# brdav/refign

Measured on AMD Instinct MI355X. Metric: image-pairs/s (align+seg fwd+bwd, 1080x1920), higher is better.
Workload: dtype bf16

## Files before the change

### include/refign_hip.h

```cpp
#ifndef REFIGN_HIP_H
#define REFIGN_HIP_H

#ifdef __cplusplus
extern "C" {
#endif

#define RFN_OK 0
#define RFN_EINVAL (-1)
#define RFN_ELAUNCH (-2)
#define RFN_ENOTSUP (-3)
#define RFN_ENONDET (-4)

#define RFN_ABI_VERSION 5

typedef void* rfn_stream_t;

int rfn_abi_version(void);
const char* rfn_last_error(void);

int rfn_set_deterministic(int on);
int rfn_get_deterministic(void);

int rfn_corr_fwd_f32(const float* in1, const float* in2, float* out, int B, int C, int iH, int iW,
                     int kH, int kW, int patchH, int patchW, int padH, int padW, int dilH, int dilW,
// ... 185 lines not shown
int rfn_bn_apply_fwd(const void* x, const float* gamma, const float* beta, void* y, const double* sums, float* running_mean,
                     float* running_var, long T, int C, float eps, float momentum, int relu, int dtype, rfn_stream_t stream);
int rfn_bn_apply_fwd_ld(const void* x, const float* gamma, const float* beta, void* y, long ld_y, const double* sums,
                        float* running_mean, float* running_var, long T, int C, float eps, float momentum, int relu, int dtype,
                        rfn_stream_t stream);
int rfn_bn_stats_bwd(const void* x, const void* grad_y, const double* fwd_sums, const float* gamma, const float* beta,
                     float* bwd_sums, long T, int C, float eps, int relu, int dtype, rfn_stream_t stream);
int rfn_bn_apply_bwd(const void* x, const void* grad_y, const double* fwd_sums, const float* bwd_sums, const float* gamma,
                     const float* beta, void* grad_x, long T, int C, float eps, int relu, int dtype, rfn_stream_t stream);
int rfn_bn_train_fwd(const void* x, const float* gamma, const float* beta, void* y, double* sums, float* running_mean,
                     float* running_var, long T, int C, float eps, float momentum, int relu, int dtype,
                     rfn_stream_t stream);
int rfn_bn_train_bwd(const void* x, const void* grad_y, const double* fwd_sums, const float* gamma, const float* beta,
                     void* grad_x, float* bwd_sums, long T, int C, float eps, int relu, int dtype, rfn_stream_t stream);

int rfn_upsample_ce(const void* logits, const long* target, const float* weight, float* grad_lo, double* loss_sum, int B,
                    int C, int h, int w, int H, int W, int ignore_index, int dtype, int round16, rfn_stream_t stream);

int rfn_slide_argmax_confmat(const void* crop_logits, int dtype, int B, int C, int h, int w, const int* boxes, int nbox, int H,
                             int W, const long* target, int ignore_index, unsigned char* labels, long* confmat,
                             rfn_stream_t stream);

int rfn_gemm_nt_o32(const void* X, const void* W, const float* bias, const float* res, const float* rowscale,
                    int rows_per_sample, int act, float* Y, long M, long N, long K, long ldx, long ldw, long ldy,
                    rfn_stream_t stream);
int rfn_conv2d_nhwc_o32(const void* X, const void* W, const float* bias, int act, float* Y, int B, int H, int Wd, int C, int N,
                        int KH, int KW, int stride, int pad, int dil, long ldw, long ldy, int transposed,
                        rfn_stream_t stream);
int rfn_conv2d_nhwc_dgrad(const void* GY, const void* Wt, void* DX, int B, int H, int W, int C, int N, int KH, int KW,
                          int stride, int pad, int dil, long ldw, long ldy, int dtype, rfn_stream_t stream);
int rfn_conv2d_nhwc_wgrad(const void* GY, const void* X, float* P, float* grad_bias, int B, int H, int W, int C, int N, int KH,
                          int KW, int stride, int pad, int dil, long ldg, long Kpad, int rows_per_slab, int accumulate,
                          int dtype, rfn_stream_t stream);

int rfn_dacs_mix_jitter(const float* src, const float* trg, const long* gt_src, const long* pseudo_label,
                        const float* pseudo_weight, float* mixed_img, long* mixed_lbl, float* mixed_weight, double* mean_ws,
                        int B, int H, int W, const long* class_bits, const int* jitter_on, const int* order,
                        const float* factor, const float* hue, const float* mean3, const float* std3,
                        rfn_stream_t stream);
int rfn_dacs_blur(const float* x, float* tmp, float* y, int B, int C, int H, int W, int ksize_y, int ksize_x, const int* blur_on,
                  const double* sigma_y, const double* sigma_x, rfn_stream_t stream);

int rfn_crop_label_hist_u8(const void* label, int H, int W, const int* boxes, int K, int* hist, rfn_stream_t stream);
int rfn_crop_flip_norm_u8(const void* image, const void* label, int C, int H, int W, int top, int left, int h, int w, int flip,
                          const float* mean3, const float* std3, float* out_image, long* out_label, rfn_stream_t stream);

int rfn_resize_crop_flip_norm_u8(const void* image_hwc, int H, int W, int Hd, int Wd, const int* bounds_x, const int* coef_x, int kmax_x,
                                 const int* bounds_y, const int* coef_y, int kmax_y, int top, int left, int h, int w, int flip,
                                 const float* mean3, const float* std3, float* out_image, rfn_stream_t stream);
int rfn_resize_u8(const void* image_hwc, int H, int W, int Hd, int Wd, const int* bounds_x, const int* coef_x, int kmax_x,
                  const int* bounds_y, const int* coef_y, int kmax_y, void* out_chw, rfn_stream_t stream);
int rfn_resize_nearest_u8(const void* label, int H, int W, int Hd, int Wd, const int* ytab, const int* xtab, void* out,
                          rfn_stream_t stream);

int rfn_resize_filter_u8(const void* image_hwc, int H, int W, int Hd, int Wd, int filter, const int* bounds_x, const int* coef_x,
                         int kmax_x, const int* bounds_y, const int* coef_y, int kmax_y, void* out_chw, rfn_stream_t stream);
int rfn_resize_filter_crop_flip_norm_pad_u8(const void* image_hwc, int H, int W, int Hd, int Wd, int filter, const int* bounds_x,
                                            const int* coef_x, int kmax_x, const int* bounds_y, const int* coef_y, int kmax_y, int top,
                                            int left, int h, int w, int flip, const float* mean3, const float* std3, float* out_image,
                                            int Hf, int Wf, rfn_stream_t stream);

int rfn_sparse_epe_f32(const float* flow, const float* conf, const float* pts_src, const float* pts_trg, const int* offsets, int B,
                       int h, int w, double* rows, rfn_stream_t stream);

int rfn_gemm_nt_f8(const void* X8, const void* W8, const float* wscale, float x_scale, const void* bias, const void* res,
                   const float* rowscale, int rows_per_sample, int act, void* Y, int out_f8, float out_q, long M, long N,
                   long K, long ldx, long ldw, long ldy, rfn_stream_t stream);
int rfn_quant_rows_f8(const void* table, int nchunks, rfn_stream_t stream);
int rfn_quant_f8(const void* x_bf16, void* y8, long n, float q, rfn_stream_t stream);
int rfn_layernorm_fwd_f8(const void* x_bf16, const float* gamma, const float* beta, void* y8, long rows, int C, float eps,
                         float out_q, rfn_stream_t stream);
int rfn_dwconv3x3_gelu_nhwc_fwd_f8(const void* x8, const float* weight, const float* bias, void* y8, int B, int H, int W, int C,
                                   float x_scale, float out_q, rfn_stream_t stream);
int rfn_attn_pack_f8(const void* kv8, long batch_stride, long row_stride, int B, int heads, int Nkv, int nst, void* pack,
                     rfn_stream_t stream);
int rfn_attn_fwd_f8(const void* q8, long q_batch_stride, long q_row_stride, const void* pack, void* o8, long o_batch_stride,
                    long o_row_stride, int B, int heads, int Nq, int Nkv, int nst, float scale, float q_scale, float k_scale,
                    float v_scale, float out_q, rfn_stream_t stream);

unsigned long rfn_bn_stats_det_workspace_bytes(long T, int C);
int rfn_bn_stats_fwd_det(const void* x, double* sums, void* workspace, long T, int C, int dtype, rfn_stream_t stream);
int rfn_bn_stats_bwd_det(const void* x, const void* grad_y, const double* fwd_sums, const float* gamma, const float* beta,
                         float* bwd_sums, void* workspace, long T, int C, float eps, int relu, int dtype, rfn_stream_t stream);
unsigned long rfn_dwconv3x3_stats_det_workspace_bytes(int B, int H, int W, int C, int dilation);
int rfn_dwconv3x3_nhwc_fwd_stats_det(const void* x, const float* weight, const float* bias, void* y, double* sums, void* workspace,
                                     int B, int H, int W, int C, int dilation, int dtype, rfn_stream_t stream);
int rfn_dwconv3x3_nhwc_stats_det(const void* x, const float* weight, const float* bias, double* sums, void* workspace, int B, int H,
                                 int W, int C, int dilation, int dtype, rfn_stream_t stream);
int rfn_attn_bwd_dkv_det(const void* K, const void* V, long kv_batch_stride, long kv_row_stride, const void* q_rpack,
                         const void* q_tpack, const void* do_rpack, const void* do_tpack, const float* lse2,
                         const float* delta, float* accT, void* dKV, int B, int heads, int Nq, int Nkv, int nqblk, int nqpad,
                         int nkpad, int blocks_per_chunk, float scale, int dtype, rfn_stream_t stream);
unsigned long rfn_dacs_mix_jitter_det_workspace_bytes(int H, int W);
int rfn_dacs_mix_jitter_det(const float* src, const float* trg, const long* gt_src, const long* pseudo_label,
                            const float* pseudo_weight, float* mixed_img, long* mixed_lbl, float* mixed_weight, double* mean_ws,
                            int B, int H, int W, const long* class_bits, const int* jitter_on, const int* order,
                            const float* factor, const float* hue, const float* mean3, const float* std3,
                            rfn_stream_t stream);
unsigned long rfn_upsample_ce_det_workspace_bytes(int B, int C, int H, int W);
int rfn_upsample_ce_det(const void* logits, const long* target, const float* weight, float* grad_lo, double* loss_sum,
                        void* workspace, int B, int C, int h, int w, int H, int W, int ignore_index, int dtype, int round16,
                        rfn_stream_t stream);
int rfn_upsample_bilinear2d_bwd(const void* grad_out, void* grad_in, long planes, int h, int w, int H, int W, float scale_y,
                                float scale_x, int dtype, rfn_stream_t stream);

int rfn_steplog_gather(const void* const* ptrs, const int* dtypes, int n, double* row, rfn_stream_t stream);
int rfn_grad_sqnorm_groups(const float* flat, long n, const long* chunks, int nchunks, int ngroups, double* partials,
                           double* out, rfn_stream_t stream);

int rfn_grad_clip_coef(const double* sqnorms, int ngroups, float max_norm, float* coef, rfn_stream_t stream);
int rfn_grad_scale_f32(float* grads, long n, const float* coef, rfn_stream_t stream);
int rfn_grad_clamp_f32(float* grads, long n, float clip_value, rfn_stream_t stream);
int rfn_amp_unscale_sqnorm_groups_f32(float* grads, long n, const long* chunks, int nchunks, int ngroups, const float* scale,
                                      float* found_inf, double* partials, double* out, rfn_stream_t stream);

int rfn_flowsynth_flow_f32(const float* theta, int kind, const float* bumps, int n_bumps, const float* field, int h, int w,
                           float* flow, int* count, rfn_stream_t stream);
int rfn_flowsynth_warp_f32(const float* image, const float* flow, const int* count, int h, int w, int top, int left, int ch, int cw,
                           double min_fraction_valid, float* out_image, float* out_flow, void* out_mask, rfn_stream_t stream);
int rfn_gaussian_blur_f32(const float* src, const float* taps, int ntaps, int planes, int h, int w, double* tmp, float* dst,
                          rfn_stream_t stream);

int rfn_flowloss_block_pixels(void);
int rfn_flowloss_fwd_f32(const float* gt_flow, int B, int H, int W, const long* levels, const double* weights, int nlevels,
                         int loss_type, float delta, double* partials, int nblocks, float* loss_out, double* counts,
                         rfn_stream_t stream);
int rfn_flowloss_bwd_f32(const float* gt_flow, int B, int H, int W, const long* levels, const double* weights, int nlevels,
                         int loss_type, float delta, const double* counts, const float* grad_out, rfn_stream_t stream);
int rfn_multi_adam_f32(const void* table, int nchunks, const float* group_args, int ngroups, rfn_stream_t stream);
int rfn_multi_adam_amp_f32(const void* table, int nchunks, const double* group_args, int ngroups, const float* found_inf,
                           const float* step, rfn_stream_t stream);

int rfn_photometric_record_words(void);
int rfn_photometric_gray_sums_u8(const void* image, const void* records, int B, int h, int w, unsigned long* sums,
                                 rfn_stream_t stream);
int rfn_photometric_apply_u8(const void* image, const void* records, const unsigned long* sums, int B, int h, int w, float* out,
                             rfn_stream_t stream);

int rfn_rotate_nearest_u8(const void* src, int C, int H, int W, int a0, int a1, int a2, int a3, int a4, int a5, int fill,
                          void* out, void* outside, rfn_stream_t stream);
int rfn_photometric_gray_sums_geom_u8(const void* image, const void* records, const void* geom, int B, int H, int W, int h, int w,
                                      unsigned long* sums, rfn_stream_t stream);
int rfn_photometric_apply_geom_u8(const void* image, const void* records, const void* geom, const unsigned long* sums, int B, int H,
                                  int W, int h, int w, float* out, rfn_stream_t stream);

unsigned long rfn_warp_bwd_det_workspace_bytes(int B, int C, int H, int W, int want_grad_x, int want_grad_flow);
int rfn_warp_bwd_det_f32(const float* x, const float* flow, const float* grad_out, float* grad_x, float* grad_flow,
                         void* workspace, int B, int C, int H, int W, rfn_stream_t stream);
int rfn_corr_bwd_gather_f32(const float* in1, const float* in2, const float* grad_out, float* grad_in1,
                            float* grad_in2, int B, int C, int iH, int iW, int kH, int kW, int patchH, int patchW,
                            int padH, int padW, int dilH, int dilW, int dpH, int dpW, int dH, int dW,
                            rfn_stream_t stream);

#ifdef __cplusplus
}
#endif
#endif
```

### refign_amd/seg.py

```python
import math
import os
import random
from functools import partial, wraps
from typing import Callable, List, Optional, Union

import torch
import torch.nn as nn
import torch.nn.functional as F

from . import f8 as _f8
from . import linear as _linear
from . import determinism, mfma
from ._tensor import const_tensor
from ._tensor import DTYPE_CODE as _CE_DT
from .align import BaseHead
from .conv import Conv2d, patch_conv_tokens
from .layernorm import LayerNorm
from .layers import MLP, ConvBNReLU, DropPath
from .linear import Linear
from .upcat import upsample_concat
from .upsample import interpolate_bilinear

_MIT = {
    'mit_b0': ([32, 64, 160, 256], [2, 2, 2, 2]),
    'mit_b1': ([64, 128, 320, 512], [2, 2, 2, 2]),
    'mit_b2': ([64, 128, 320, 512], [3, 4, 6, 3]),
    'mit_b3': ([64, 128, 320, 512], [3, 4, 18, 3]),
    'mit_b4': ([64, 128, 320, 512], [3, 8, 27, 3]),
    'mit_b5': ([64, 128, 320, 512], [3, 6, 40, 3]),
}
_MIT_HEADS = [1, 2, 5, 8]
_MIT_SR = [8, 4, 2, 1]


_GRAD_READY_CB = None


class _GradMark(torch.autograd.Function):

    @staticmethod
    def forward(ctx, x, tag):
        ctx.tag = tag
        return x.view_as(x)

    @staticmethod
    def backward(ctx, g):
        cb = _GRAD_READY_CB
        if cb is not None:
            cb(ctx.tag)
        return g, None


def grad_mark(x, tag):
    return _GradMark.apply(x, tag) if (torch.is_grad_enabled() and x.requires_grad) else x


class DWConv(nn.Module):

    def __init__(self, dim=768):
        super().__init__()
        self.dwconv = nn.Conv2d(dim, dim, 3, 1, 1, bias=True, groups=dim)

    def forward(self, x, H, W):
        B, N, C = x.shape
        if x.is_cuda and C % 8 == 0:
            from .dwconv import dwconv3x3_tokens
            return dwconv3x3_tokens(x, self.dwconv.weight, self.dwconv.bias, H, W)
        y = self.dwconv(x.transpose(1, 2).reshape(B, C, H, W))
        return y.flatten(2).transpose(1, 2)


class Mlp(nn.Module):

    def __init__(self, in_features, hidden_features=None, out_features=None, act_layer=nn.GELU, drop=0.):
        super().__init__()
        out_features = out_features or in_features
        hidden_features = hidden_features or in_features
        self.fc1 = Linear(in_features, hidden_features)
        self.dwconv = DWConv(hidden_features)
        self.act = act_layer()
        self.fc2 = Linear(hidden_features, out_features)
        self.drop = nn.Dropout(drop)

    def forward(self, x, H, W, res=None, rowscale=None):
        if x.is_cuda and not torch.is_grad_enabled() and x.dtype in (torch.bfloat16, torch.float16) and type(self.act) is nn.GELU \
                and self.act.approximate == 'none' and self.drop.p == 0. and type(self.fc1) is Linear and not _f8.active():
            from .dwconv import ffn_fc1_dw_gelu
            a = ffn_fc1_dw_gelu(x, self.fc1, self.dwconv.dwconv, H, W)
            if a is not None:
                return self.fc2(a, res=res, rowscale=rowscale) if res is not None else self.fc2(a)
        x = self.fc1(x)
        if x.is_cuda and x.shape[-1] % 8 == 0 and type(self.act) is nn.GELU and self.act.approximate == 'none':
            from .dwconv import dwconv3x3_gelu_tokens
            dw = self.dwconv.dwconv
            if torch.is_grad_enabled() and x.requires_grad and self.drop.p == 0. and x.dtype in (torch.bfloat16, torch.float16) \
                    and os.environ.get("RFN_FUSED_GELU_BWD", "1") == "1":
                a, z = dwconv3x3_gelu_tokens(x, dw.weight, dw.bias, H, W, with_z=True)
                if res is not None:
                    return self.fc2(a, res=res, rowscale=rowscale, z=z)
                return self.fc2(a, z=z)
            x = self.drop(dwconv3x3_gelu_tokens(x, dw.weight, dw.bias, H, W))
        else:
            x = self.drop(self.act(self.dwconv(x, H, W)))
        if res is not None and self.drop.p == 0.:
            return self.fc2(x, res=res, rowscale=rowscale)
        y = self.drop(self.fc2(x))
        return y if res is None else _residual(res, y, rowscale)


_SDPA_BACKEND = None
_FUSED_UPCAT = True


def _fused_upcat_here():
    return _FUSED_UPCAT
_SR_AS_LINEAR = True
_KV_FUSED = True


class Attention(nn.Module):

    def __init__(self, dim, num_heads=8, qkv_bias=False, qk_scale=None, attn_drop=0., proj_drop=0., sr_ratio=1):
        super().__init__()
        assert dim % num_heads == 0, f'dim {dim} should be divided by num_heads {num_heads}.'
        self.dim, self.num_heads = dim, num_heads
        self.scale = qk_scale or (dim // num_heads) ** -0.5
        self.q = Linear(dim, dim, bias=qkv_bias)
        self.kv = Linear(dim, dim * 2, bias=qkv_bias)
        self.attn_drop = nn.Dropout(attn_drop)
        self.proj = Linear(dim, dim)
        self.proj_drop = nn.Dropout(proj_drop)
        self.sr_ratio = sr_ratio
        if sr_ratio > 1:
            self.sr = Conv2d(dim, dim, kernel_size=sr_ratio, stride=sr_ratio)
            self.norm = LayerNorm(dim)

    def forward(self, x, H, W, res=None, rowscale=None, x_kv=None):
        B, N, C = x.shape
        h, d = self.num_heads, C // self.num_heads
        q = self.q(x)
        if x_kv is not None:
            x = x_kv
        p = self.attn_drop.p if self.training else 0.0
        if _KV_FUSED and not torch.is_grad_enabled() and x.is_cuda and d == 64 and p == 0.0 and _SDPA_BACKEND is None \
                and q.dtype == x.dtype and type(self.kv) is Linear and not _f8.active() \
                and (self.sr_ratio == 1 or (_SR_AS_LINEAR and type(self.norm) is LayerNorm)):
            packs = mfma.kv_packs(x, H, W, self.sr if self.sr_ratio > 1 else None, self.norm if self.sr_ratio > 1 else None,
                                  self.kv)
            o = mfma.attention_packed(q, packs, h, self.scale) if packs is not None else None
            if o is not None:
                return self._project(o, res, rowscale)
        if self.sr_ratio > 1:
            r = patch_conv_tokens(x, H, W, self.sr) if _SR_AS_LINEAR else None
            if r is None:
                r = self.sr(x.transpose(1, 2).reshape(B, C, H, W)).flatten(2).transpose(1, 2)
            x = self.norm(r)
        kv = self.kv(x)
        o = mfma.attention(q, kv, h, self.scale) if (d == 64 and p == 0.0 and _SDPA_BACKEND is None) else None
        if o is None and q.is_cuda and q.dtype == torch.float32 and p == 0.0 and _SDPA_BACKEND is None:
            from . import split32
            if split32.usable(q, kv) and d in (32, 64):
                o = split32.attention(q, kv, h, self.scale)
        if o is None:
            mfma.note_library("sdpa", q, kv)
            q = q.view(B, N, h, d).transpose(1, 2)
# ... 325 lines not shown

class SegFormerHead(BaseHead):

    os: int = 4

    def __init__(self, in_channels: List[int], in_index: Union[List[int], int], num_classes: int,
                 input_transform: Optional[str] = None, channels: int = 256, dropout_ratio: float = 0.1):
        super().__init__(num_classes, in_index, input_transform)
        self.in_channels = in_channels
        c1, c2, c3, c4 = in_channels
        self.linear_c4 = MLP(input_dim=c4, embed_dim=channels)
        self.linear_c3 = MLP(input_dim=c3, embed_dim=channels)
        self.linear_c2 = MLP(input_dim=c2, embed_dim=channels)
        self.linear_c1 = MLP(input_dim=c1, embed_dim=channels)
        self.linear_fuse = ConvBNReLU(channels * 4, channels, kernel_size=1, norm_layer=nn.BatchNorm2d)
        self.linear_pred = nn.Conv2d(channels, num_classes, kernel_size=1)
        self.dropout = nn.Dropout2d(dropout_ratio) if dropout_ratio > 0 else None
        nn.init.normal_(self.linear_pred.weight, mean=0, std=0.01)
        nn.init.zeros_(self.linear_pred.bias)
        _mmseg_init(self)

    def forward(self, inputs):
        c1, c2, c3, c4 = inputs
        size = c1.shape[2:]

        feats = [c4, c3, c2, c1]
        toks = [layer(f) for layer, f in zip((self.linear_c4, self.linear_c3, self.linear_c2, self.linear_c1), feats)]
        cat = upsample_concat(toks, [f.shape[2:] for f in feats], size) if _fused_upcat_here() else None
        if cat is None:
            parts = []
            for t, f in zip(toks, feats):
                n, _, h, w = f.shape
                t = t.transpose(1, 2).reshape(n, -1, h, w)
                parts.append(t if (h, w) == tuple(size) else _up(t, size))
            cat = torch.cat(parts, dim=1)
        y = self.linear_fuse(cat)
        if self.dropout is not None:
            y = self.dropout(y)
        return _class_logits(self.linear_pred, y)


_PREDRAWN_CROPS = []
_DEVICE_CROPS = []


class DeviceBox:

    def __init__(self, off, h, w, divisible):
        self.off, self.h, self.w, self.divisible = off, int(h), int(w), int(divisible)

    def _idx(self, n, which, scale=1):
        return torch.arange(n, device=self.off.device) + self.off[which] // scale

    def crop(self, x):
        return x.index_select(-2, self._idx(self.h, 0)).index_select(-1, self._idx(self.w, 1))

    def mask(self, H, W, scale, like):
        assert self.divisible % int(scale) == 0
        hs, ws = int(self.h / scale), int(self.w / scale)
        ry = torch.arange(H, device=self.off.device) - self.off[0] // int(scale)
        rx = torch.arange(W, device=self.off.device) - self.off[1] // int(scale)
        m = ((ry >= 0) & (ry < hs))[:, None] & ((rx >= 0) & (rx < ws))[None, :]
        return m.to(like.dtype).view(1, 1, H, W)

    def insert(self, patch, size, scale):
        assert self.divisible % int(scale) == 0
        H, W = size
        hs, ws = patch.shape[-2:]
        ry = torch.arange(H, device=self.off.device) - self.off[0] // int(scale)
        rx = torch.arange(W, device=self.off.device) - self.off[1] // int(scale)
        ry = torch.where((ry >= 0) & (ry < hs), ry, torch.full_like(ry, hs))
        rx = torch.where((rx >= 0) & (rx < ws), rx, torch.full_like(rx, ws))
        return F.pad(patch, (0, 1, 0, 1)).index_select(-2, ry).index_select(-1, rx)


def push_device_crop(off, divisible):
    _DEVICE_CROPS.append((off, divisible))


def draw_crop_offsets(H, W, crop_size, divisible=1):
    if H == crop_size[-2] and W == crop_size[-1]:
        return None
    oy = random.randrange(0, int((max(H - crop_size[-2], 0) + 1) // divisible)) * divisible
    ox = random.randrange(0, int((max(W - crop_size[-1], 0) + 1) // divisible)) * divisible
    return int(oy), int(ox)


def predraw_crop(H, W, crop_size, divisible=1):
    _PREDRAWN_CROPS.append(((H, W, tuple(crop_size), divisible), draw_crop_offsets(H, W, crop_size, divisible)))


def extract_crop(img, crop_size, divisible=1):
    H, W = img.shape[-2:]
    assert crop_size[0] > 0 and crop_size[1] > 0
    if _DEVICE_CROPS:
        off, div = _DEVICE_CROPS.pop(0)
        assert div == divisible, (div, divisible)
        box = DeviceBox(off, crop_size[0], crop_size[1], divisible)
        return box.crop(img), [box]
    if _PREDRAWN_CROPS:
        key, off = _PREDRAWN_CROPS.pop(0)
        assert key == (H, W, tuple(crop_size), divisible), (key, (H, W, tuple(crop_size), divisible))
    else:
        off = draw_crop_offsets(H, W, crop_size, divisible)
    if off is None:
        return (0, H, 0, W)
    oy, ox = off
    y1, y2, x1, x2 = int(oy), int(oy + crop_size[0]), int(ox), int(ox + crop_size[1])
    return img[:, :, y1:y2, x1:x2], [[y1, y2, x1, x2]]


def scale_box(box, scale):
    return tuple(int(v / scale) for v in box)


def hr_crop_slice(crop_box, scale):
    y1, y2, x1, x2 = scale_box(crop_box, scale)
    return slice(y1, y2), slice(x1, x2)


def extract_slide_crop(img, crop_size):
    hc, wc = crop_size
    hs, ws = hc // 2, wc // 2
    H, W = img.shape[-2:]
    crops, boxes = [], []
    for iy in range(max(H - hc + hs - 1, 0) // hs + 1):
        for ix in range(max(W - wc + ws - 1, 0) // ws + 1):
            y2, x2 = min(iy * hs + hc, H), min(ix * ws + wc, W)
            y1, x1 = max(y2 - hc, 0), max(x2 - wc, 0)
            crops.append(img[:, :, y1:y2, x1:x2])
            boxes.append([y1, y2, x1, x2])
    return torch.cat(crops, dim=0), boxes


def hrda_backbone(self, head_os: int, is_teacher: bool = False) -> Callable:
    def deco(fn: Callable) -> Callable:
        @wraps(fn)
        def inner(x, *args, **kwargs):
            lr = F.interpolate(x, scale_factor=0.5, mode='bilinear', align_corners=False)
            size = lr.shape[-2:]
            if self.training and not is_teacher:
                hr, boxes = extract_crop(x, size, head_os * 2.0)
            else:
                hr, boxes = extract_slide_crop(x, size)
            nl, nh = lr.shape[0], hr.shape[0]
            feats = fn(torch.cat((lr, hr)), *args, **kwargs)
            lr_feats, hr_feats = zip(*(torch.split(f, [nl, nh]) for f in feats))
            return lr_feats, hr_feats, boxes
        return inner
    return deco


_REJOIN = True


def _rejoin(a, b):
    if _REJOIN and (not torch.is_grad_enabled() or not (a.requires_grad or b.requires_grad)) and a.dim() >= 2 \
            and a.dtype == b.dtype \
            and a.shape[1:] == b.shape[1:] and a.stride() == b.stride() and a.device == b.device \
            and a.untyped_storage().data_ptr() == b.untyped_storage().data_ptr() \
            and b.storage_offset() == a.storage_offset() + a.shape[0] * a.stride(0):
        dense = sorted(zip(a.stride()[1:], a.shape[1:]))
        run = 1
        for st, n in dense:
            if n != 1 and st != run:
                return torch.cat((a, b))
            run *= n
        if a.stride(0) == run:
            return a.as_strided((a.shape[0] + b.shape[0], *a.shape[1:]), a.stride(), a.storage_offset())
    return torch.cat((a, b))


def hrda_head(self, hrda_scale_attention: nn.Module, head_os: int, is_teacher: bool = False) -> Callable:
    def deco(fn: Callable) -> Callable:
        @wraps(fn)
        def inner(inp, *args, **kwargs):
            lr_feats, hr_feats, boxes = inp
            att = torch.sigmoid(hrda_scale_attention(lr_feats))
            nl, nh = lr_feats[0].shape[0], hr_feats[0].shape[0]
            seg = fn([_rejoin(*p) for p in zip(lr_feats, hr_feats)], *args, **kwargs)
            lr_seg, hr_seg = torch.split(seg, [nl, nh])
            if self.training and not is_teacher and isinstance(boxes[0], DeviceBox):
                box = boxes[0]
                att = att * box.mask(lr_seg.shape[2], lr_seg.shape[3], 2.0 * head_os, lr_seg)
                up_lr = interpolate_bilinear((1 - att) * lr_seg, scale_factor=2)
                up_att = interpolate_bilinear(att, scale_factor=2)
                inserted = box.insert(hr_seg, up_lr.shape[2:], head_os)
                return up_att * inserted + up_lr, defer_logits(hr_seg, (box.h, box.w), fused_ce_consumer(self)), box
            if self.training and not is_teacher:
                box = boxes[0]
                crop_size = (box[1] - box[0], box[3] - box[2])
                mask = lr_seg.new_zeros([nl, 1, *lr_seg.shape[2:]])
                sy, sx = hr_crop_slice(box, 2.0 * head_os)
                mask[:, :, sy, sx] = 1
                att = att * mask
                up_lr = interpolate_bilinear((1 - att) * lr_seg, scale_factor=2)
                up_att = interpolate_bilinear(att, scale_factor=2)
                inserted = torch.zeros_like(up_lr)
                sy, sx = hr_crop_slice(box, head_os)
                inserted[:, :, sy, sx] = hr_seg
                hr_logits = defer_logits(hr_seg, crop_size, fused_ce_consumer(self))
                return up_att * inserted + up_lr, hr_logits, box
            up_lr = F.interpolate((1 - att) * lr_seg, scale_factor=2, mode='bilinear', align_corners=False)
            for i in range(len(boxes)):
                boxes[i] = scale_box(boxes[i], head_os)
            Hh, Ww = max(b[1] for b in boxes), max(b[3] for b in boxes)
            preds = lr_seg.new_zeros((nl, self.num_classes, Hh, Ww))
            count = lr_seg.new_zeros((nl, 1, Hh, Ww))
            for i, (y1, y2, x1, x2) in enumerate(boxes):
                preds[:, :, y1:y2, x1:x2] += hr_seg[i * nl:(i + 1) * nl]
                count[:, :, y1:y2, x1:x2] += 1
            up_att = F.interpolate(att, scale_factor=2, mode='bilinear', align_corners=False)
            return up_att * (preds / count) + up_lr
        return inner
    return deco


_FUSED_CE = True


def mark_fused_ce_consumer(module, loss):
    module._rfn_fused_ce_consumer = type(loss) is PixelWeightedCrossEntropyLoss
    return module._rfn_fused_ce_consumer


def fused_ce_consumer(module):
    return bool(getattr(module, "_rfn_fused_ce_consumer", False))


class DeferredUpsample:

    def __init__(self, logits, size):
        self.logits, self.size = logits, (int(size[0]), int(size[1]))

    def materialize(self):
        return _up_logits(self.logits, self.size)

    @property
    def shape(self):
        return torch.Size((*self.logits.shape[:2], *self.size))

    @classmethod
    def __torch_function__(cls, func, types, args=(), kwargs=None):
        conv = lambda a: a.materialize() if isinstance(a, DeferredUpsample) else a
        return func(*[conv(a) for a in args], **{k: conv(v) for k, v in (kwargs or {}).items()})


def defer_logits(logits, size, consumer_is_fused_ce=False):
    if _FUSED_CE and consumer_is_fused_ce and logits.is_cuda and logits.dim() == 4 and logits.dtype in _CE_DT and logits.shape[1] <= 19 \
            and size[0] >= 2 * logits.shape[2] and size[1] >= 2 * logits.shape[3] and torch.is_grad_enabled():
        return DeferredUpsample(logits, size)
    return _up_logits(logits, size)


class _UpsampleCEFn(torch.autograd.Function):

    @staticmethod
    def forward(ctx, logits, target, weight, size, ignore_index):
        from . import _lib
        from ._tensor import ptr
        B, C, h, w = logits.shape
        H, W = size
        lg = logits.contiguous()
        tg = target.contiguous()
        wt = None if weight is None else weight.to(torch.float32).contiguous()
        if tg.dtype != torch.int64 or tuple(tg.shape) != (B, H, W) or (wt is not None and tuple(wt.shape) != (B, H, W)):
            raise RuntimeError("upsample_ce: target (B, H, W) int64 / weight (B, H, W) expected")
        grad = torch.empty((B, C, h, w), dtype=torch.float32, device=lg.device)
        total = torch.empty(64, dtype=torch.float64, device=lg.device)
        rc = None
        lib = _lib.load_library()
        if determinism.enabled():
            from ._tensor import workspace
            ws = workspace(lib.rfn_upsample_ce_det_workspace_bytes(B, C, H, W), lg.device)
            _lib.call("rfn_upsample_ce_det", lg.device, ptr(lg), ptr(tg), ptr(wt), ptr(grad), ptr(total), ptr(ws), B, C, h, w,
                      H, W, int(ignore_index), _CE_DT[lg.dtype], 1)
            ctx.save_for_backward(grad)
            ctx.npix, ctx.dtype = float(B * H * W), logits.dtype
            return (total[0] / ctx.npix).to(torch.float32)
        _lib.call("rfn_upsample_ce", lg.device, ptr(lg), ptr(tg), ptr(wt), ptr(grad), ptr(total), B, C, h, w, H, W,
                  int(ignore_index), _CE_DT[lg.dtype], 1)
        ctx.save_for_backward(grad)
        ctx.npix, ctx.dtype = float(B * H * W), logits.dtype
        return (total.sum() / ctx.npix).to(torch.float32)

    @staticmethod
    def backward(ctx, g):
        (grad,) = ctx.saved_tensors
        return (grad * (g.to(torch.float32) / ctx.npix)).to(ctx.dtype), None, None, None, None


class PixelWeightedCrossEntropyLoss(nn.Module):

    def __init__(self, ignore_index: int = 255) -> None:
        super().__init__()
        self.ignore_index = ignore_index

    def forward(self, input, target, pixel_weight=None):
        if isinstance(input, DeferredUpsample):
            if pixel_weight is not None:
                assert pixel_weight.dim() == target.dim()
            return _UpsampleCEFn.apply(input.logits, target, pixel_weight, input.size, self.ignore_index)
        loss = F.cross_entropy(input, target, ignore_index=self.ignore_index, reduction='none')
        if pixel_weight is not None:
            assert pixel_weight.dim() == loss.dim()
            loss = loss * pixel_weight.to(loss.dtype)
        return loss.mean()
```

Measured before the change: 17.42.

## Fuse HRDA attention-merge tail into single forward and backward kernels

Adds HIP kernels that take the raw scale-attention logits, lr and hr segmentation maps and produce the merged high-resolution logits in one pass. Sigmoid, crop mask, bilinear upsampling, crop insertion and blend are computed per output element instead of through a chain of separate PyTorch elementwise and interpolate ops. A matching fused backward kernel does the same for training, plus a fused sliding-window merge for the teacher/eval path. This removes many full-resolution intermediate tensors and kernel launches, at the cost of per-pixel recomputation, float64 accumulation in backward, and float32 channels-last output.

```diff
diff --git a/include/refign_hip.h b/include/refign_hip.h
--- a/include/refign_hip.h
+++ b/include/refign_hip.h
@@ -361,6 +361,17 @@
                             int padH, int padW, int dilH, int dilW, int dpH, int dpW, int dH, int dW,
                             rfn_stream_t stream);
 
+int rfn_hrda_merge_slide(const void* a, const long* a_strides, const void* lr, const long* lr_strides, const void* hr,
+                         const long* hr_strides, const int* boxes, int nb, float* out, int nl, int K, int h, int w, int hc, int wc,
+                         int dtype, int* accepted, rfn_stream_t stream);
+int rfn_hrda_fuse_crop_fwd(const void* a, const long* a_strides, const void* lr, const long* lr_strides, const void* hr,
+                           const long* hr_strides, const long* off, float* out, int n, int K, int h, int w, int hc, int wc, int mh,
+                           int mw, int div_mask, int div_ins, int dtype, rfn_stream_t stream);
+int rfn_hrda_fuse_crop_bwd(const float* grad_out, const long* g_strides, const void* a, const long* a_strides, const void* lr,
+                           const long* lr_strides, const void* hr, const long* hr_strides, const long* off, void* grad_a,
+                           void* grad_lr, void* grad_hr, int n, int K, int h, int w, int hc, int wc, int mh, int mw, int div_mask,
+                           int div_ins, int dtype, rfn_stream_t stream);
+
 #ifdef __cplusplus
 }
 #endif
diff --git a/refign_amd/csrc/hrdatail.hip b/refign_amd/csrc/hrdatail.hip
--- /dev/null
+++ b/refign_amd/csrc/hrdatail.hip
@@ -0,0 +1,291 @@
+#include <hip/hip_bf16.h>
+
+#include "bilinear.h"
+#include "common.h"
+#include "elem.h"
+
+namespace rfn {
+
+constexpr int kHrdaMaxBoxes = 16;
+
+struct HrdaMap {
+  const void* p;
+  long sn, sc, sh, sw;
+};
+struct HrdaBoxes {
+  int nb;
+  int y1[kHrdaMaxBoxes], y2[kHrdaMaxBoxes], x1[kHrdaMaxBoxes], x2[kHrdaMaxBoxes];
+};
+
+template <typename T>
+__device__ __forceinline__ float hrda_ld(const HrdaMap& m, long n, int c, long y, long x) {
+  return ldf<T>(reinterpret_cast<const T*>(m.p) + n * m.sn + c * m.sc + y * m.sh + x * m.sw);
+}
+
+__device__ __forceinline__ float hrda_blend(float ly, float lx, float v00, float v01, float v10, float v11) {
+  const float hy = 1.0f - ly, hx = 1.0f - lx;
+  return hy * (hx * v00 + lx * v01) + ly * (hx * v10 + lx * v11);
+}
+
+__device__ __forceinline__ float hrda_mul_add(float a, float b, float c) {
+#pragma clang fp contract(off)
+  const float p = a * b;
+  return p + c;
+}
+
+template <typename T>
+__device__ __forceinline__ void hrda_tap(float av, float lv, bool masked, bool inmask, float& att, float& tl) {
+  const float s = round_to<T>(1.0f / (1.0f + expf(-av)));
+  att = !masked || inmask ? s : s * 0.0f;
+  const float om = round_to<T>(1.0f - att);
+  tl = round_to<T>(om * lv);
+}
+
+struct HrdaCrop {
+  long my0, mx0, iy0, ix0;
+};
+__device__ __forceinline__ HrdaCrop hrda_crop(const long* __restrict__ off, int div_mask, int div_ins) {
+  const long oy = off[0], ox = off[1];
+  return HrdaCrop{oy / div_mask, ox / div_mask, oy / div_ins, ox / div_ins};
+}
+
+template <typename T, int MODE>
+__global__ __launch_bounds__(256) void hrda_merge_fwd_kernel(HrdaMap a, HrdaMap lr, HrdaMap hr, HrdaBoxes bx,
+                                                             const long* __restrict__ off, float* __restrict__ out, int nl, int K,
+                                                             int h, int w, int hc, int wc, int mh, int mw, int div_mask,
+                                                             int div_ins, long total) {
+  const long idx = (long)blockIdx.x * 256 + threadIdx.x;
+  if (idx >= total) return;
+  const int H = 2 * h, W = 2 * w;
+  const int c = (int)(idx % K);
+  long pix = idx / K;
+  const int X = (int)(pix % W);
+  pix /= W;
+  const int Y = (int)(pix % H);
+  const long n = pix / H;
+  int y0, y1, x0, x1;
+  float ly, lx;
+  up_src(Y, 0.5f, h, y0, y1, ly);
+  up_src(X, 0.5f, w, x0, x1, lx);
+  HrdaCrop cr{0, 0, 0, 0};
+  if constexpr (MODE == 1) cr = hrda_crop(off, div_mask, div_ins);
+  const int ys[2] = {y0, y1}, xs[2] = {x0, x1};
+  float att[4], tl[4];
+#pragma unroll
+  for (int i = 0; i < 2; ++i) {
+#pragma unroll
+    for (int j = 0; j < 2; ++j) {
+      const long ry = ys[i] - cr.my0, rx = xs[j] - cr.mx0;
+      const bool inmask = ry >= 0 && ry < mh && rx >= 0 && rx < mw;
+      hrda_tap<T>(hrda_ld<T>(a, n, c, ys[i], xs[j]), hrda_ld<T>(lr, n, c, ys[i], xs[j]), MODE == 1, inmask, att[2 * i + j],
+                  tl[2 * i + j]);
+    }
+  }
+  const float ua = hrda_blend(ly, lx, att[0], att[1], att[2], att[3]);
+  const float ul = hrda_blend(ly, lx, tl[0], tl[1], tl[2], tl[3]);
+  float q;
+  if constexpr (MODE == 0) {
+    float acc = 0.0f, cnt = 0.0f;
+    for (int i = 0; i < bx.nb; ++i) {
+      if (Y >= bx.y1[i] && Y < bx.y2[i] && X >= bx.x1[i] && X < bx.x2[i]) {
+        acc = round_to<T>(acc + hrda_ld<T>(hr, (long)i * nl + n, c, Y - bx.y1[i], X - bx.x1[i]));
+        cnt = cnt + 1.0f;
+      }
+    }
+    q = round_to<T>(acc / cnt);
+  } else {
+    const long ry = Y - cr.iy0, rx = X - cr.ix0;
+    q = ry >= 0 && ry < hc && rx >= 0 && rx < wc ? hrda_ld<T>(hr, n, c, ry, rx) : 0.0f;
+  }
+  out[idx] = hrda_mul_add(ua, q, ul);
+}
+
+__device__ __forceinline__ double hrda_sigmoid64(float a) { return 1.0 / (1.0 + exp(-(double)a)); }
+
+template <typename T>
+__device__ __forceinline__ void hrda_crop_bwd_lr(const HrdaMap& g, const HrdaMap& a, const HrdaMap& lr, const HrdaMap& hr,
+                                                 const long* __restrict__ off, T* __restrict__ g_a, T* __restrict__ g_lr, int K,
+                                                 int h, int w, int hc, int wc, int mh, int mw, int div_mask, int div_ins,
+                                                 long idx) {
+  const int H = 2 * h, W = 2 * w;
+  const int c = (int)(idx % K);
+  long pix = idx / K;
+  const int x = (int)(pix % w);
+  pix /= w;
+  const int y = (int)(pix % h);
+  const long n = pix / h;
+  const HrdaCrop cr = hrda_crop(off, div_mask, div_ins);
+  double t = 0.0, u = 0.0;
+  const int Ylo = max(0, 2 * y - 1), Yhi = min(H - 1, 2 * y + 2), Xlo = max(0, 2 * x - 1), Xhi = min(W - 1, 2 * x + 2);
+  for (int Y = Ylo; Y <= Yhi; ++Y) {
+    int i0, i1;
+    float l;
+    up_src(Y, 0.5f, h, i0, i1, l);
+    const float wy = (i0 == y ? 1.0f - l : 0.0f) + (i1 == y ? l : 0.0f);
+    if (wy == 0.0f) continue;
+    const long ry = Y - cr.iy0;
+    for (int X = Xlo; X <= Xhi; ++X) {
+      up_src(X, 0.5f, w, i0, i1, l);
+      const float wx = (i0 == x ? 1.0f - l : 0.0f) + (i1 == x ? l : 0.0f);
+      if (wx == 0.0f) continue;
+      const double gw = (double)wy * (double)wx * (double)hrda_ld<float>(g, n, c, Y, X);
+      u += gw;
+      const long rx = X - cr.ix0;
+      if (ry >= 0 && ry < hc && rx >= 0 && rx < wc) t += gw * (double)hrda_ld<T>(hr, n, c, ry, rx);
+    }
+  }
+  const long my = y - cr.my0, mx = x - cr.mx0;
+  const bool inmask = my >= 0 && my < mh && mx >= 0 && mx < mw;
+  const double s = hrda_sigmoid64(hrda_ld<T>(a, n, c, y, x)), lv = (double)hrda_ld<T>(lr, n, c, y, x);
+  const double att = inmask ? s : 0.0;
+  stf(g_lr + idx, (float)((1.0 - att) * u));
+  stf(g_a + idx, (float)(inmask ? (t - lv * u) * s * (1.0 - s) : 0.0));
+}
+
+template <typename T>
+__device__ __forceinline__ void hrda_crop_bwd_hr(const HrdaMap& g, const HrdaMap& a, const long* __restrict__ off,
+                                                 T* __restrict__ g_hr, int K, int h, int w, int hc, int wc, int mh, int mw,
+                                                 int div_mask, int div_ins, long idx) {
+  const int H = 2 * h, W = 2 * w;
+  const int c = (int)(idx % K);
+  long pix = idx / K;
+  const int xh = (int)(pix % wc);
+  pix /= wc;
+  const int yh = (int)(pix % hc);
+  const long n = pix / hc;
+  const HrdaCrop cr = hrda_crop(off, div_mask, div_ins);
+  const long Yl = cr.iy0 + yh, Xl = cr.ix0 + xh;
+  double r = 0.0;
+  if (Yl >= 0 && Yl < H && Xl >= 0 && Xl < W) {
+    const int Y = (int)Yl, X = (int)Xl;
+    int y0, y1, x0, x1;
+    float ly, lx;
+    up_src(Y, 0.5f, h, y0, y1, ly);
+    up_src(X, 0.5f, w, x0, x1, lx);
+    const int ys[2] = {y0, y1}, xs[2] = {x0, x1};
+    const double wys[2] = {1.0 - (double)ly, (double)ly}, wxs[2] = {1.0 - (double)lx, (double)lx};
+    double ua = 0.0;
+#pragma unroll
+    for (int i = 0; i < 2; ++i) {
+#pragma unroll
+      for (int j = 0; j < 2; ++j) {
+        const long my = ys[i] - cr.my0, mx = xs[j] - cr.mx0;
+        if (my >= 0 && my < mh && mx >= 0 && mx < mw) ua += wys[i] * wxs[j] * hrda_sigmoid64(hrda_ld<T>(a, n, c, ys[i], xs[j]));
+      }
+    }
+    r = ua * (double)hrda_ld<float>(g, n, c, Y, X);
+  }
+  stf(g_hr + idx, (float)r);
+}
+
+template <typename T>
+__global__ __launch_bounds__(256) void hrda_crop_bwd_kernel(HrdaMap g, HrdaMap a, HrdaMap lr, HrdaMap hr,
+                                                            const long* __restrict__ off, T* __restrict__ g_a,
+                                                            T* __restrict__ g_lr, T* __restrict__ g_hr, int K, int h, int w, int hc,
+                                                            int wc, int mh, int mw, int div_mask, int div_ins, long tot_lr,
+                                                            long tot_hr) {
+  const long idx = (long)blockIdx.x * 256 + threadIdx.x;
+  if (idx < tot_lr) hrda_crop_bwd_lr<T>(g, a, lr, hr, off, g_a, g_lr, K, h, w, hc, wc, mh, mw, div_mask, div_ins, idx);
+  else if (idx < tot_lr + tot_hr) hrda_crop_bwd_hr<T>(g, a, off, g_hr, K, h, w, hc, wc, mh, mw, div_mask, div_ins, idx - tot_lr);
+}
+
+static HrdaMap hrda_map(const void* p, const long* st) { return HrdaMap{p, st[0], st[1], st[2], st[3]}; }
+
+static bool hrda_boxes_cover(const int* b, int nb, int rows, int cols) {
+  int ye[2 * kHrdaMaxBoxes + 2], xe[2 * kHrdaMaxBoxes + 2], ny = 0, nx = 0;
+  ye[ny++] = 0;
+  xe[nx++] = 0;
+  for (int i = 0; i < nb; ++i) {
+    ye[ny++] = b[4 * i];
+    ye[ny++] = b[4 * i + 1];
+    xe[nx++] = b[4 * i + 2];
+    xe[nx++] = b[4 * i + 3];
+  }
+  for (int iy = 0; iy < ny; ++iy) {
+    if (ye[iy] < 0 || ye[iy] >= rows) continue;
+    for (int ix = 0; ix < nx; ++ix) {
+      if (xe[ix] < 0 || xe[ix] >= cols) continue;
+      bool in = false;
+      for (int i = 0; i < nb && !in; ++i)
+        in = ye[iy] >= b[4 * i] && ye[iy] < b[4 * i + 1] && xe[ix] >= b[4 * i + 2] && xe[ix] < b[4 * i + 3];
+      if (!in) return false;
+    }
+  }
+  return true;
+}
+
+}
+
+using namespace rfn;
+
+extern "C" {
+
+int rfn_hrda_merge_slide(const void* a, const long* a_strides, const void* lr, const long* lr_strides, const void* hr,
+                         const long* hr_strides, const int* boxes, int nb, float* out, int nl, int K, int h, int w, int hc, int wc,
+                         int dtype, int* accepted, rfn_stream_t stream) {
+  RFN_REQUIRE(a && a_strides && lr && lr_strides && hr && hr_strides && boxes && out && accepted && nb > 0 && nl > 0 && K > 0 &&
+                  h > 0 && w > 0 && hc > 0 && wc > 0,
+              "rfn_hrda_merge_slide: bad arguments");
+  RFN_REQUIRE(dtype == 1, "rfn_hrda_merge_slide: bf16 operands only (dtype 1, got %d)", dtype);
+  const long total = (long)nl * 2 * h * 2 * w * K;
+  RFN_REQUIRE(total / 256 < 0x7fffffffL && h < (1 << 29) && w < (1 << 29), "rfn_hrda_merge_slide: too large");
+  *accepted = 0;
+  if (nb > kHrdaMaxBoxes) return RFN_OK;
+  HrdaBoxes bx;
+  int ymax = 0, xmax = 0;
+  for (int i = 0; i < nb; ++i) {
+    const int y1 = boxes[4 * i], y2 = boxes[4 * i + 1], x1 = boxes[4 * i + 2], x2 = boxes[4 * i + 3];
+    if (y1 < 0 || x1 < 0 || y2 - y1 != hc || x2 - x1 != wc || y2 > 2 * h || x2 > 2 * w) return RFN_OK;
+    bx.y1[i] = y1; bx.y2[i] = y2; bx.x1[i] = x1; bx.x2[i] = x2;
+    ymax = y2 > ymax ? y2 : ymax;
+    xmax = x2 > xmax ? x2 : xmax;
+  }
+  bx.nb = nb;
+  if (ymax != 2 * h || xmax != 2 * w || !hrda_boxes_cover(boxes, nb, 2 * h, 2 * w)) return RFN_OK;
+  *accepted = 1;
+  const HrdaMap ma = hrda_map(a, a_strides), ml = hrda_map(lr, lr_strides), mh_ = hrda_map(hr, hr_strides);
+  using T = __hip_bfloat16;
+  hipLaunchKernelGGL((hrda_merge_fwd_kernel<T, 0>), dim3(cdiv(total, 256)), dim3(256), 0, (hipStream_t)stream, ma, ml, mh_, bx,
+                     (const long*)nullptr, out, nl, K, h, w, hc, wc, 0, 0, 1, 1, total);
+  return check_launch("hrda_merge_fwd_kernel<slide>");
+}
+
+int rfn_hrda_fuse_crop_fwd(const void* a, const long* a_strides, const void* lr, const long* lr_strides, const void* hr,
+                           const long* hr_strides, const long* off, float* out, int n, int K, int h, int w, int hc, int wc, int mh,
+                           int mw, int div_mask, int div_ins, int dtype, rfn_stream_t stream) {
+  RFN_REQUIRE(a && a_strides && lr && lr_strides && hr && hr_strides && off && out && n > 0 && K > 0 && h > 0 && w > 0 && hc > 0 &&
+                  wc > 0 && mh >= 0 && mw >= 0 && div_mask > 0 && div_ins > 0,
+              "rfn_hrda_fuse_crop_fwd: bad arguments");
+  RFN_REQUIRE(dtype == 1, "rfn_hrda_fuse_crop_fwd: bf16 operands only (dtype 1, got %d)", dtype);
+  const long total = (long)n * 2 * h * 2 * w * K;
+  RFN_REQUIRE(total / 256 < 0x7fffffffL && h < (1 << 29) && w < (1 << 29), "rfn_hrda_fuse_crop_fwd: too large");
+  const HrdaMap ma = hrda_map(a, a_strides), ml = hrda_map(lr, lr_strides), mh_ = hrda_map(hr, hr_strides);
+  HrdaBoxes bx;
+  bx.nb = 0;
+  using T = __hip_bfloat16;
+  hipLaunchKernelGGL((hrda_merge_fwd_kernel<T, 1>), dim3(cdiv(total, 256)), dim3(256), 0, (hipStream_t)stream, ma, ml, mh_, bx,
+                     off, out, n, K, h, w, hc, wc, mh, mw, div_mask, div_ins, total);
+  return check_launch("hrda_merge_fwd_kernel<crop>");
+}
+
+int rfn_hrda_fuse_crop_bwd(const float* grad_out, const long* g_strides, const void* a, const long* a_strides, const void* lr,
+                           const long* lr_strides, const void* hr, const long* hr_strides, const long* off, void* grad_a,
+                           void* grad_lr, void* grad_hr, int n, int K, int h, int w, int hc, int wc, int mh, int mw, int div_mask,
+                           int div_ins, int dtype, rfn_stream_t stream) {
+  RFN_REQUIRE(grad_out && g_strides && a && a_strides && lr && lr_strides && hr && hr_strides && off && grad_a && grad_lr &&
+                  grad_hr && n > 0 && K > 0 && h > 0 && w > 0 && hc > 0 && wc > 0 && mh >= 0 && mw >= 0 && div_mask > 0 &&
+                  div_ins > 0,
+              "rfn_hrda_fuse_crop_bwd: bad arguments");
+  RFN_REQUIRE(dtype == 1, "rfn_hrda_fuse_crop_bwd: bf16 operands only (dtype 1, got %d)", dtype);
+  const long tot_lr = (long)n * h * w * K, tot_hr = (long)n * hc * wc * K;
+  RFN_REQUIRE((tot_lr + tot_hr) / 256 < 0x7fffffffL && h < (1 << 29) && w < (1 << 29),
+              "rfn_hrda_fuse_crop_bwd: too large");
+  const HrdaMap mg = hrda_map(grad_out, g_strides), ma = hrda_map(a, a_strides), ml = hrda_map(lr, lr_strides),
+                mh_ = hrda_map(hr, hr_strides);
+  using T = __hip_bfloat16;
+  hipLaunchKernelGGL((hrda_crop_bwd_kernel<T>), dim3(cdiv(tot_lr + tot_hr, 256)), dim3(256), 0, (hipStream_t)stream, mg, ma, ml,
+                     mh_, off, (T*)grad_a, (T*)grad_lr, (T*)grad_hr, K, h, w, hc, wc, mh, mw, div_mask, div_ins, tot_lr, tot_hr);
+  return check_launch("hrda_crop_bwd_kernel");
+}
+
+}
diff --git a/refign_amd/hrdatail.py b/refign_amd/hrdatail.py
--- /dev/null
+++ b/refign_amd/hrdatail.py
@@ -0,0 +1,70 @@
+import ctypes
+
+import torch
+
+from . import _lib
+from ._tensor import DTYPE_CODE, ptr
+
+_L4 = ctypes.c_long * 4
+
+
+def _strides(t):
+    return _L4(*t.stride())
+
+
+def usable(a, lr_seg, hr_seg):
+    return (a.is_cuda and lr_seg.is_cuda and hr_seg.is_cuda and a.dim() == 4 and hr_seg.dim() == 4 and a.shape == lr_seg.shape
+            and hr_seg.shape[1] == a.shape[1] and a.dtype == lr_seg.dtype == hr_seg.dtype == torch.bfloat16
+            and torch.is_autocast_enabled())
+
+
+def merge_slide(a, lr_seg, hr_seg, boxes):
+    nl, K, h, w = lr_seg.shape
+    nb = len(boxes)
+    if nb == 0 or hr_seg.shape[0] != nb * nl or not usable(a, lr_seg, hr_seg) or \
+            (torch.is_grad_enabled() and (a.requires_grad or lr_seg.requires_grad or hr_seg.requires_grad)):
+        return None
+    hc, wc = hr_seg.shape[2:]
+    out = torch.empty((nl, 2 * h, 2 * w, K), dtype=torch.float32, device=a.device)
+    accepted = ctypes.c_int(0)
+    flat = (ctypes.c_int * (4 * nb))(*[int(v) for b in boxes for v in b])
+    _lib.call("rfn_hrda_merge_slide", a.device, ptr(a), _strides(a), ptr(lr_seg), _strides(lr_seg), ptr(hr_seg), _strides(hr_seg),
+              flat, nb, ptr(out), nl, K, h, w, hc, wc, DTYPE_CODE[a.dtype], ctypes.byref(accepted))
+    return out.permute(0, 3, 1, 2) if accepted.value else None
+
+
+class _FuseCrop(torch.autograd.Function):
+    @staticmethod
+    def forward(ctx, a, lr_seg, hr_seg, off, geom):
+        n, K, h, w = lr_seg.shape
+        hc, wc = hr_seg.shape[2:]
+        out = torch.empty((n, 2 * h, 2 * w, K), dtype=torch.float32, device=a.device)
+        _lib.call("rfn_hrda_fuse_crop_fwd", a.device, ptr(a), _strides(a), ptr(lr_seg), _strides(lr_seg), ptr(hr_seg),
+                  _strides(hr_seg), ptr(off), ptr(out), n, K, h, w, hc, wc, *geom, DTYPE_CODE[a.dtype])
+        ctx.save_for_backward(a, lr_seg, hr_seg, off)
+        ctx.geom = geom
+        return out.permute(0, 3, 1, 2)
+
+    @staticmethod
+    def backward(ctx, g):
+        a, lr_seg, hr_seg, off = ctx.saved_tensors
+        n, K, h, w = lr_seg.shape
+        hc, wc = hr_seg.shape[2:]
+        if g.dtype != torch.float32:
+            g = g.float()
+        g_a = torch.empty((n, h, w, K), dtype=a.dtype, device=a.device)
+        g_lr = torch.empty((n, h, w, K), dtype=a.dtype, device=a.device)
+        g_hr = torch.empty((n, hc, wc, K), dtype=a.dtype, device=a.device)
+        _lib.call("rfn_hrda_fuse_crop_bwd", a.device, ptr(g), _strides(g), ptr(a), _strides(a), ptr(lr_seg), _strides(lr_seg),
+                  ptr(hr_seg), _strides(hr_seg), ptr(off), ptr(g_a), ptr(g_lr), ptr(g_hr), n, K, h, w, hc, wc, *ctx.geom,
+                  DTYPE_CODE[a.dtype])
+        return g_a.permute(0, 3, 1, 2), g_lr.permute(0, 3, 1, 2), g_hr.permute(0, 3, 1, 2), None, None
+
+
+def fuse_crop(a, lr_seg, hr_seg, box, head_os):
+    os_ = int(head_os)
+    if not (usable(a, lr_seg, hr_seg) and hr_seg.shape[0] == a.shape[0] and os_ == head_os and box.off.is_cuda
+            and box.off.dtype == torch.long and box.off.numel() == 2 and box.off.is_contiguous() and box.divisible % (2 * os_) == 0):
+        return None
+    geom = (int(box.h / (2.0 * os_)), int(box.w / (2.0 * os_)), 2 * os_, os_)
+    return _FuseCrop.apply(a, lr_seg, hr_seg, box.off, geom)
diff --git a/refign_amd/seg.py b/refign_amd/seg.py
--- a/refign_amd/seg.py
+++ b/refign_amd/seg.py
@@ -10,7 +10,7 @@
 
 from . import f8 as _f8
 from . import linear as _linear
-from . import determinism, mfma
+from . import determinism, hrdatail, mfma
 from ._tensor import const_tensor
 from ._tensor import DTYPE_CODE as _CE_DT
 from .align import BaseHead
@@ -642,6 +642,7 @@
 
 
 _REJOIN = True
+_HRDA_TAIL_FUSED = True
 
 
 def _rejoin(a, b):
@@ -666,18 +667,23 @@
         @wraps(fn)
         def inner(inp, *args, **kwargs):
             lr_feats, hr_feats, boxes = inp
-            att = torch.sigmoid(hrda_scale_attention(lr_feats))
+            att_logits = hrda_scale_attention(lr_feats)
             nl, nh = lr_feats[0].shape[0], hr_feats[0].shape[0]
             seg = fn([_rejoin(*p) for p in zip(lr_feats, hr_feats)], *args, **kwargs)
             lr_seg, hr_seg = torch.split(seg, [nl, nh])
             if self.training and not is_teacher and isinstance(boxes[0], DeviceBox):
                 box = boxes[0]
+                fused = hrdatail.fuse_crop(att_logits, lr_seg, hr_seg, box, head_os) if _HRDA_TAIL_FUSED else None
+                if fused is not None:
+                    return fused, defer_logits(hr_seg, (box.h, box.w), fused_ce_consumer(self)), box
+                att = torch.sigmoid(att_logits)
                 att = att * box.mask(lr_seg.shape[2], lr_seg.shape[3], 2.0 * head_os, lr_seg)
                 up_lr = interpolate_bilinear((1 - att) * lr_seg, scale_factor=2)
                 up_att = interpolate_bilinear(att, scale_factor=2)
                 inserted = box.insert(hr_seg, up_lr.shape[2:], head_os)
                 return up_att * inserted + up_lr, defer_logits(hr_seg, (box.h, box.w), fused_ce_consumer(self)), box
             if self.training and not is_teacher:
+                att = torch.sigmoid(att_logits)
                 box = boxes[0]
                 crop_size = (box[1] - box[0], box[3] - box[2])
                 mask = lr_seg.new_zeros([nl, 1, *lr_seg.shape[2:]])
@@ -691,9 +697,13 @@
                 inserted[:, :, sy, sx] = hr_seg
                 hr_logits = defer_logits(hr_seg, crop_size, fused_ce_consumer(self))
                 return up_att * inserted + up_lr, hr_logits, box
-            up_lr = F.interpolate((1 - att) * lr_seg, scale_factor=2, mode='bilinear', align_corners=False)
             for i in range(len(boxes)):
                 boxes[i] = scale_box(boxes[i], head_os)
+            fused = hrdatail.merge_slide(att_logits, lr_seg, hr_seg, boxes) if _HRDA_TAIL_FUSED else None
+            if fused is not None:
+                return fused
+            att = torch.sigmoid(att_logits)
+            up_lr = F.interpolate((1 - att) * lr_seg, scale_factor=2, mode='bilinear', align_corners=False)
             Hh, Ww = max(b[1] for b in boxes), max(b[3] for b in boxes)
             preds = lr_seg.new_zeros((nl, self.num_classes, Hh, Ww))
             count = lr_seg.new_zeros((nl, 1, Hh, Ww))
```

Measured after the change: 17.66, median of 6. +1.4%, better.
